# gk969/stm32-speech-recognition

Hardware: AMD Instinct MI355X
Metric: utterances/sec (256-frame, 100 templates) (higher is better)
Workload: dtype int32

## Files before the change

### stm32_speech_recognition_amd/csrc/k_mfcc.hip

```cpp
#include "sr_fft_dev.h"

#include <type_traits>

#ifndef SR_MEL_CHUNKED
#define SR_MEL_CHUNKED 1
#endif

namespace sr {

constexpr int kMfccWaves = 4;
constexpr int kFramesPerWave = 16, kFramesPerWaveMid = 4, kFramesPerWaveSmall = 1;
#ifndef SR_MAG_TAB_BINS
#define SR_MAG_TAB_BINS 8
#endif
constexpr int mfcc_tab_bins(int fpw) { return fpw == kFramesPerWave ? SR_MAG_TAB_BINS : 0; }
static_assert(SR_MAG_TAB_BINS == 0 || SR_MAG_TAB_BINS == 4 || SR_MAG_TAB_BINS == 8, "table bins per lane");
#ifndef SR_MFCC_PIPE
#define SR_MFCC_PIPE 1
#endif
#ifndef SR_MFCC_PIPE_PEEL
#define SR_MFCC_PIPE_PEEL 1
#endif
#ifndef SR_MFCC_PIPE_VMCNT
#define SR_MFCC_PIPE_VMCNT (SR_MFCC_PIPE_PEEL ? 3 : 0)
#endif
static_assert(SR_MFCC_PIPE_VMCNT == 0 || (SR_MFCC_PIPE_VMCNT == 3 && SR_MFCC_PIPE_PEEL), "younger loads counted by the wait");
constexpr bool mfcc_pipelined(int fpw) { return SR_MFCC_PIPE && mfcc_tab_bins(fpw) == 8; }
#ifndef SR_MFCC_TM_REGS
#define SR_MFCC_TM_REGS 1
#endif
#ifdef SR_INJECT_LDS_RACE
#undef SR_MFCC_TM_REGS
#define SR_MFCC_TM_REGS 0
#endif
constexpr bool mfcc_tm_regs(int fpw) { return SR_MFCC_TM_REGS && mfcc_pipelined(fpw); }
constexpr int kMelPad = kMel + 1;
__device__ __forceinline__ constexpr int mel_chunk_word(int j) { return 256 * ((j >> 2) & 1) + 4 * ((j >> 3) ^ (4 * ((j >> 2) & 1))) + (j & 3); }
#ifndef SR_MFCC_PREFIX_TID
#define SR_MFCC_PREFIX_TID 1
#endif
__device__ __forceinline__ constexpr int mel_prefix_word(int j)
{
#if SR_MFCC_PREFIX_TID
    return 64 * (j & 7) + (j >> 3);
#elif SR_MEL_CHUNKED
    return mel_chunk_word(j);
#else
    return j;
#endif
}
#pragma clang diagnostic push
#pragma clang diagnostic ignored "-Winline-asm"
__device__ __forceinline__ void mel_prefix_store(uint32_t base, const uint32_t (&pe)[8], const uint32_t (&po)[8])
{
    static_assert(kBins == 512, "the offsets below are written out for two halves of 512 words");
    asm volatile("s_mov_b32 m0, %16\n\ts_nop 0\n\t"
                 "ds_write_addtid_b32 %0\n\tds_write_addtid_b32 %1 offset:256\n\tds_write_addtid_b32 %2 offset:512\n\t"
                 "ds_write_addtid_b32 %3 offset:768\n\tds_write_addtid_b32 %4 offset:1024\n\tds_write_addtid_b32 %5 offset:1280\n\t"
                 "ds_write_addtid_b32 %6 offset:1536\n\tds_write_addtid_b32 %7 offset:1792\n\t"
                 "ds_write_addtid_b32 %8 offset:2048\n\tds_write_addtid_b32 %9 offset:2304\n\tds_write_addtid_b32 %10 offset:2560\n\t"
                 "ds_write_addtid_b32 %11 offset:2816\n\tds_write_addtid_b32 %12 offset:3072\n\tds_write_addtid_b32 %13 offset:3328\n\t"
                 "ds_write_addtid_b32 %14 offset:3584\n\tds_write_addtid_b32 %15 offset:3840"
                 :
                 : "v"(pe[0]), "v"(pe[1]), "v"(pe[2]), "v"(pe[3]), "v"(pe[4]), "v"(pe[5]), "v"(pe[6]), "v"(pe[7]), "v"(po[0]),
                   "v"(po[1]), "v"(po[2]), "v"(po[3]), "v"(po[4]), "v"(po[5]), "v"(po[6]), "v"(po[7]), "s"(base)
                 : "m0", "memory");
}
#pragma clang diagnostic pop
constexpr int mfcc_wave_lds_words(int fpw) { return kXchgWords + fpw * kMelPad + 64; }

template <typename Base>
struct MfccTabArgs : Base {
    const uint16_t *mag_q;
    uint32_t mag_table_off;
};
template <typename Base>
constexpr int mfcc_feat_kind<MfccTabArgs<Base>> = mfcc_feat_kind<Base>;
template <typename Base>
static MfccTabArgs<Base> mfcc_tab_args(const Base &b, const MfccMagTab &tab)
{
    MfccTabArgs<Base> r;
    static_cast<Base &>(r) = b;
    r.mag_q = tab.mag_q;
    r.mag_table_off = tab.mag_table_off;
    return r;
}

template <int kFPW, typename Args = MfccTabArgs<MfccArgs>>
__global__ void __launch_bounds__(64 * kMfccWaves, 4) k_mfcc(const Args a)
{
    constexpr int kFeat = mfcc_feat_kind<Args>;
    constexpr uint32_t kFeatW = (kFeat == SR_FEAT_FFT || kFeat == SR_FEAT_MAG) ? kBins : kMel;
    constexpr int kWaveLdsWords = mfcc_wave_lds_words(kFPW);
    constexpr int kTabBins = mfcc_tab_bins(kFPW);
    constexpr bool kPipe = mfcc_pipelined(kFPW);
    constexpr bool kTmRegs = mfcc_tm_regs(kFPW);
    extern __shared__ __attribute__((aligned(16))) uint32_t smem[];
    __shared__ uint32_t s_dctM[kCoef * kMelPad];
    __shared__ int s_dctS[kCoef * kMelPad];
    __shared__ u32x4 s_tw3[kTw3Row * 4], s_tw5[8 * 64];
    __shared__ u32x4 s_tm[4 * 64];
    const int lane = threadIdx.x & 63, w = __builtin_amdgcn_readfirstlane(threadIdx.x >> 6);
    uint32_t *buf = smem + w * kWaveLdsWords;
    uint32_t *xw = buf;
    uint32_t *powb = buf + kXchgWords, *moff = powb + kFPW * kMelPad;
    const uint32_t buf_lds = (uint32_t)(uintptr_t)(const __attribute__((address_space(3))) uint32_t *)buf;
    (void)buf_lds;

    for (int i = threadIdx.x; i < kCoef * kMel; i += blockDim.x) {
        const int c = a.t.dct[i], o = (i / kMel) * kMelPad + i % kMel;
        s_dctM[o] = (uint32_t)(((c < 0 ? -c : c) * 262144 + 99) / 100);
        s_dctS[o] = (c > 0) - (c < 0);
    }
    __syncthreads();

    LaneTw tw;
    load_lane_tw(a.t, lane, tw);
    real_leg_tw(tw);
    if (w == 0 && lane < 4) {
        const uint32_t *f = &tw.s3[0][0][0];
#pragma unroll
        for (int c = 0; c < 8; c++) s_tw3[lane * kTw3Row + c] = u32x4{f[4 * c], f[4 * c + 1], f[4 * c + 2], f[4 * c + 3]};
    }
    if (w == 1 % kMfccWaves) store_tw32(s_tw5, lane, tw.s5);
    u32x4 tm_r[4];
    if constexpr (kTmRegs) {
#pragma unroll
        for (int c = 0; c < 2; c++) {
            tm_r[c] = *(const u32x4 *)(a.t.tri_even_m + 8 * lane + 4 * c);
            tm_r[c + 2] = *(const u32x4 *)(a.t.tri_odd_m + 8 * lane + 4 * c);
        }
    }
#ifndef SR_INJECT_LDS_RACE
    if (!kTmRegs && w == 2 % kMfccWaves) {
#pragma unroll
        for (int c = 0; c < 2; c++) {
            s_tm[64 * c + lane] = *(const u32x4 *)(a.t.tri_even_m + 8 * lane + 4 * c);
            s_tm[64 * (c + 2) + lane] = *(const u32x4 *)(a.t.tri_odd_m + 8 * lane + 4 * c);
        }
    }
#endif
    __syncthreads();
#ifdef SR_INJECT_LDS_RACE
    if (w == 2 % kMfccWaves) {
#if SR_INJECT_LDS_RACE >= 2
        __builtin_amdgcn_s_sleep(127);
#endif
#pragma unroll
        for (int c = 0; c < 2; c++) {
            s_tm[64 * c + lane] = *(const u32x4 *)(a.t.tri_even_m + 8 * lane + 4 * c);
            s_tm[64 * (c + 2) + lane] = *(const u32x4 *)(a.t.tri_odd_m + 8 * lane + 4 * c);
        }
    }
#endif
    int hamm_m[3];
#pragma unroll
    for (int k = 0; k < 3; k++) hamm_m[k] = (lane + 64 * k < kFrameLen) ? hamm_fused_multiplier(a.t.hamm[lane + 64 * k]) : 0;
    int f_lo = 0, p_hi = 0, p_lo = 0, x_hi = 0, x_lo = 0;
    if (lane < kMel) {
        const int h = lane;
        f_lo = (h == 0) ? 0 : (int)a.t.tri_cen[h - 1];
        const int f_hi = (h == kMel - 1) ? kBins : (int)a.t.tri_cen[h + 1];
        const int ih = f_hi - 1, il = f_lo ? f_lo - 1 : 0, half = (h & 1) ? kBins : 0;
        p_hi = half + mel_prefix_word(ih), x_hi = (ih >> 3) > 0 ? (ih >> 3) - 1 : 0;
        p_lo = half + mel_prefix_word(il), x_lo = (il >> 3) > 0 ? (il >> 3) - 1 : 0;
    }
    const uint64_t mag_p = (uint64_t)a.mag_q;
    const u32x4 mag_rs = {(uint32_t)mag_p, (uint32_t)(mag_p >> 32) | (2u << 16), kMagTabEntries, 0x00027000u};
    const uint32_t tw_off = 32u * (uint32_t)lane;
#if SR_MEL_CHUNKED
    const int e_base = mel_chunk_word(lane);
    constexpr int kEs = 32, kEh = 128;
    const int c0 = mel_chunk_word(8 * lane), c1 = mel_chunk_word(8 * lane + 4);
#else
    const int e_base = lane;
    constexpr int kEs = 64, kEh = 256;
    const int c0 = 8 * lane, c1 = 8 * lane + 4;
#endif

    uint32_t item = blockIdx.x;
    uint32_t nx_nfrm = 0;
    int nx_mid = 0, nx_seg0 = 0;
    if (item < a.n_items) {
        const sr_vad_rec *rec = a.vad + item / a.tiles;
        nx_nfrm = rec->frm_num;
        nx_mid = (int)rec->atap.mid_val;
        nx_seg0 = rec->seg[0];
    }
    for (; item < a.n_items; item += gridDim.x) {
        const uint32_t b = item / a.tiles, tile = item - b * a.tiles;
        const uint32_t nfrm = nx_nfrm;
        const int mid = nx_mid, seg0 = nx_seg0;
        if (item + gridDim.x < a.n_items) {
            const sr_vad_rec *rec = a.vad + (item + gridDim.x) / a.tiles;
            nx_nfrm = rec->frm_num;
            nx_mid = (int)rec->atap.mid_val;
            nx_seg0 = rec->seg[0];
        }
        const uint16_t *row = a.pcm + (uint64_t)b * a.pcm_stride;
        int16_t *out = a.mfcc + (uint64_t)b * a.max_frames * kCoef;
        const uint32_t f0 = tile * (kMfccWaves * kFPW) + w * kFPW;
        uint32_t *frow = nullptr;
        if constexpr (kFeat != 0) frow = a.feat + (uint64_t)b * a.max_frames * kFeatW;
        uint32_t nf = 0;
        if (f0 < nfrm) nf = (nfrm - f0 < (uint32_t)kFPW) ? nfrm - f0 : (uint32_t)kFPW;

        uint32_t s_pp[3] = {0, 0, 0};
        if (nf) {
            const uint16_t *x = row + seg0 + (int)kHop * (int)f0;
#pragma unroll
            for (int k = 0; k < 3; k++) {
                const int i = lane + 64 * k;
                if (i < kFrameLen) s_pp[k] = *(const u32_align2 *)(x + i - 1);
            }
        }
        auto store_prefixes = [&](const uint32_t (&pe)[8], const uint32_t (&po)[8]) {
#if SR_MFCC_PREFIX_TID
            mel_prefix_store(buf_lds, pe, po);
#else
            *(uint4 *)(buf + c0) = make_uint4(pe[0], pe[1], pe[2], pe[3]);
            *(uint4 *)(buf + c1) = make_uint4(pe[4], pe[5], pe[6], pe[7]);
            *(uint4 *)(buf + kBins + c0) = make_uint4(po[0], po[1], po[2], po[3]);
            *(uint4 *)(buf + kBins + c1) = make_uint4(po[4], po[5], po[6], po[7]);
#endif
        };
        if constexpr (!kPipe)
        for (uint32_t fi = 0; fi < nf; fi++) {
#pragma unroll
            for (int k = 0; k < 3; k++) {
                const int i = lane + 64 * k;
                if (i < kFrameLen) k == 0 ? window_store<0>(xw, i, s_pp[k], mid, hamm_m[k]) : window_store<1>(xw, i, s_pp[k], mid, hamm_m[k]);
            }
            if (fi + 1 < nf) {
                const uint16_t *x = row + seg0 + (int)kHop * (int)(f0 + fi + 1);
#pragma unroll
                for (int k = 0; k < 3; k++) {
                    const int i = lane + 64 * k;
                    if (i < kFrameLen) s_pp[k] = *(const u32_align2 *)(x + i - 1);
                }
            }
            wave_sync();
            uint32_t v[4][4], u[4][4];
            fft_front_real160(xw, lane, tw, s_tw3, v);
            fft_exchange(buf, lane, v, u);
#pragma unroll
            for (int e4 = 0; e4 < 4; e4++) fft_pass4_dbl(u, e4, tw);
            wave_sync();
            uint32_t k5[4][4][2];
            load_tw32(s_tw5, lane, k5);
            uint32_t nn[8];
#pragma unroll
            for (int e3 = 0; e3 < 4; e3++) {
                bfly_pk_dbl<true, false, 0>(u[e3][0], u[e3][1], u[e3][2], u[e3][3], k5[e3][0][0], k5[e3][0][1], k5[e3][1][0],
                                            k5[e3][1][1], k5[e3][2][0], k5[e3][2][1], k5[e3][3][0], k5[e3][3][1]);
                if constexpr (kFeat == SR_FEAT_FFT) {
                    uint32_t *fr = frow + (f0 + fi) * kFeatW + lane + 64 * e3;
                    fr[0] = u[e3][0];
                    fr[256] = u[e3][1];
                }
                nn[2 * e3] = (uint32_t)sdot2z(u[e3][0], u[e3][0]);
                nn[2 * e3 + 1] = (uint32_t)sdot2z(u[e3][1], u[e3][1]);
            }
            const uint32_t nmax = max(max(max(max(nn[0], nn[1]), nn[2]), max(max(nn[3], nn[4]), nn[5])), max(nn[6], nn[7]));
#ifdef SR_TESTING
            const bool quiet = __builtin_expect(__builtin_amdgcn_ballot_w64(nmax > kMagSmallMax) == 0 && !a.mag_table_off, 1);
#else
            const bool quiet = __builtin_expect(__builtin_amdgcn_ballot_w64(nmax > kMagSmallMax) == 0, 1);
#endif
            u32x4 tw_e[2], tw_o[2];
            bool cheap = true;
            if (!quiet) {
#pragma unroll
                for (int c = 0; c < 2; c++) {
                    tw_e[c] = *(const u32x4 *)((const char *)a.t.tri_even32 + tw_off + 16 * c);
                    tw_o[c] = *(const u32x4 *)((const char *)a.t.tri_odd32 + tw_off + 16 * c);
                }
                cheap = __builtin_amdgcn_ballot_w64(nmax > a.mag_cheap_max) == 0;
            } else {
                asm volatile("" : "=v"(tw_e[0]), "=v"(tw_e[1]), "=v"(tw_o[0]), "=v"(tw_o[1]));
            }
            uint32_t *eb = buf + e_base;
            if (kTabBins > 0 && quiet) {
                uint32_t tq[8];
#pragma unroll
                for (int e3 = 0; e3 < 4; e3++) {
                    if constexpr (kTabBins == 8)
                        asm volatile("buffer_load_ushort %0, %1, %2, 0 idxen" : "=v"(tq[2 * e3]) : "v"(nn[2 * e3]), "s"(mag_rs));
                    asm volatile("buffer_load_ushort %0, %1, %2, 0 idxen" : "=v"(tq[2 * e3 + 1]) : "v"(nn[2 * e3 + 1]), "s"(mag_rs));
                }
                uint32_t q0s[4];
                if constexpr (kTabBins == 4) {
#pragma unroll
                    for (int e3 = 0; e3 < 4; e3++) q0s[e3] = cvt_u32(__builtin_amdgcn_sqrtf((float)(int)nn[2 * e3]) * 10.0f) << 2;
                }
                if constexpr (kTabBins == 8)
                    asm volatile("s_waitcnt vmcnt(0)" : "+v"(tq[0]), "+v"(tq[1]), "+v"(tq[2]), "+v"(tq[3]), "+v"(tq[4]), "+v"(tq[5]), "+v"(tq[6]), "+v"(tq[7]));
                else
                    asm volatile("s_waitcnt vmcnt(0)" : "+v"(tq[1]), "+v"(tq[3]), "+v"(tq[5]), "+v"(tq[7]));
#pragma unroll
                for (int e3 = 0; e3 < 4; e3++) {
                    uint32_t q0, q1 = tq[2 * e3 + 1];
                    if constexpr (kTabBins == 8) q0 = tq[2 * e3];
                    else q0 = q0s[e3];
                    if constexpr (kFeat == SR_FEAT_MAG) {
                        uint32_t *fr = frow + (f0 + fi) * kFeatW + lane + 64 * e3;
                        fr[0] = q0 >> 2;
                        fr[256] = q1 >> 2;
                    }
                    eb[kEs * e3] = umul24(q0, q0);
                    eb[kEs * e3 + kEh] = umul24(q1, q1);
                }
            } else if (cheap) {
#pragma unroll
                for (int e3 = 0; e3 < 4; e3++) {
                    const f32x2 m = f32x2{__builtin_amdgcn_sqrtf((float)(int)nn[2 * e3]), __builtin_amdgcn_sqrtf((float)(int)nn[2 * e3 + 1])} *
                                    f32x2{10.0f, 10.0f};
                    const uint32_t m0 = cvt_u32(m.x), m1 = cvt_u32(m.y);
                    if constexpr (kFeat == SR_FEAT_MAG) {
                        uint32_t *fr = frow + (f0 + fi) * kFeatW + lane + 64 * e3;
                        fr[0] = m0;
                        fr[256] = m1;
                    }
                    eb[kEs * e3] = umul24(m0, m0);
                    eb[kEs * e3 + kEh] = umul24(m1, m1);
                }
            } else {
#pragma unroll
                for (int e3 = 0; e3 < 4; e3++) {
                    const f32x2 m = sqrt_rn_int2(f32x2{(float)(int)nn[2 * e3], (float)(int)nn[2 * e3 + 1]}) * f32x2{10.0f, 10.0f};
                    const uint32_t m0 = cvt_u32(m.x), m1 = cvt_u32(m.y);
                    if constexpr (kFeat == SR_FEAT_MAG) {
                        uint32_t *fr = frow + (f0 + fi) * kFeatW + lane + 64 * e3;
                        fr[0] = m0;
                        fr[256] = m1;
                    }
                    eb[kEs * e3] = umul24(m0, m0);
                    eb[kEs * e3 + kEh] = umul24(m1, m1);
                }
            }
            wave_sync();
            uint32_t pe[8], po[8], xe, xo;
            {
                const uint4 q0 = *(const uint4 *)(buf + c0), q1 = *(const uint4 *)(buf + c1);
                const uint32_t e[8] = {q0.x, q0.y, q0.z, q0.w, q1.x, q1.y, q1.z, q1.w};
                uint32_t se = 0, so = 0;
                if (quiet) {
#pragma unroll
                    for (int c = 0; c < 2; c++) {
                        const u32x4 me = s_tm[64 * c + lane], mo = s_tm[64 * (c + 2) + lane];
#pragma unroll
                        for (int k = 0; k < 4; k++) {
                            const uint32_t es = kTabBins > 0 ? e[4 * c + k] : e[4 * c + k] << 4;
                            se += mel_term_fused(es, me[k]);
                            so += mel_term_fused(es, mo[k]);
                            pe[4 * c + k] = se;
                            po[4 * c + k] = so;
                        }
                    }
                } else {
#pragma unroll
                    for (int c = 0; c < 2; c++) {
#pragma unroll
                        for (int k = 0; k < 4; k++) {
                            se += e[4 * c + k] * tw_e[c][k] / 100u;
                            so += e[4 * c + k] * tw_o[c][k] / 100u;
                            pe[4 * c + k] = se;
                            po[4 * c + k] = so;
                        }
                    }
                }
                xe = wave_scan_incl(se);
                xo = wave_scan_incl(so);
            }
            store_prefixes(pe, po);
            buf[2 * kBins + lane] = xe;
            moff[lane] = xo;
            wave_sync();
            if (lane < kMel) {
                const uint32_t *X = (lane & 1) ? moff : buf + 2 * kBins;
                const uint32_t hi = buf[p_hi] + X[x_hi], lo = f_lo ? buf[p_lo] + X[x_lo] : 0u;
                powb[fi * kMelPad + lane] = hi - lo;
                if constexpr (kFeat == SR_FEAT_MEL) frow[(f0 + fi) * kFeatW + lane] = hi - lo;
            }
            wave_sync();
        } else {
            uint32_t mq[8] = {0, 0, 0, 0, 0, 0, 0, 0};
            bool pq = true;
            auto window = [&]() {
#pragma unroll
                for (int k = 0; k < 3; k++) {
                    const int i = lane + 64 * k;
                    if (i < kFrameLen) k == 0 ? window_store<0>(xw, i, s_pp[k], mid, hamm_m[k]) : window_store<1>(xw, i, s_pp[k], mid, hamm_m[k]);
                }
            };
            auto request = [&](uint32_t f) {
                const uint16_t *x = row + seg0 + (int)kHop * (int)(f0 + f);
#pragma unroll
                for (int k = 0; k < 3; k++) {
                    const int i = lane + 64 * k;
                    if (i < kFrameLen) s_pp[k] = *(const u32_align2 *)(x + i - 1);
                }
            };
            auto middle = [&](uint32_t fi, uint32_t (&v)[4][4], bool more) {
                uint32_t u[4][4];
                fft_exchange(buf, lane, v, u);
#pragma unroll
                for (int e4 = 0; e4 < 4; e4++) fft_pass4_dbl(u, e4, tw);
                wave_sync();
                uint32_t k5[4][4][2];
                load_tw32(s_tw5, lane, k5);
                uint32_t nn[8];
#pragma unroll
                for (int e3 = 0; e3 < 4; e3++) {
                    bfly_pk_dbl<true, false, 0>(u[e3][0], u[e3][1], u[e3][2], u[e3][3], k5[e3][0][0], k5[e3][0][1], k5[e3][1][0],
                                                k5[e3][1][1], k5[e3][2][0], k5[e3][2][1], k5[e3][3][0], k5[e3][3][1]);
                    if constexpr (kFeat == SR_FEAT_FFT) {
                        uint32_t *fr = frow + (f0 + fi) * kFeatW + lane + 64 * e3;
                        fr[0] = u[e3][0];
                        fr[256] = u[e3][1];
                    }
                    nn[2 * e3] = (uint32_t)sdot2z(u[e3][0], u[e3][0]);
                    nn[2 * e3 + 1] = (uint32_t)sdot2z(u[e3][1], u[e3][1]);
                }
                const uint32_t nmax = max(max(max(max(nn[0], nn[1]), nn[2]), max(max(nn[3], nn[4]), nn[5])), max(nn[6], nn[7]));
                if (more) {
                    wave_sync();
                    window();
                }
#ifdef SR_TESTING
                const bool quiet = __builtin_expect(__builtin_amdgcn_ballot_w64(nmax > kMagSmallMax) == 0 && !a.mag_table_off, 1);
#else
                const bool quiet = __builtin_expect(__builtin_amdgcn_ballot_w64(nmax > kMagSmallMax) == 0, 1);
#endif
                if (quiet) {
#pragma unroll
                    for (int k = 0; k < 8; k++) asm volatile("buffer_load_ushort %0, %1, %2, 0 idxen" : "=v"(mq[k]) : "v"(nn[k]), "s"(mag_rs));
                } else if (__builtin_amdgcn_ballot_w64(nmax > a.mag_cheap_max) == 0) {
#pragma unroll
                    for (int e3 = 0; e3 < 4; e3++) {
                        const f32x2 m = f32x2{__builtin_amdgcn_sqrtf((float)(int)nn[2 * e3]), __builtin_amdgcn_sqrtf((float)(int)nn[2 * e3 + 1])} *
                                        f32x2{10.0f, 10.0f};
                        mq[2 * e3] = cvt_u32(m.x);
                        mq[2 * e3 + 1] = cvt_u32(m.y);
                    }
                } else {
#pragma unroll
                    for (int e3 = 0; e3 < 4; e3++) {
                        const f32x2 m = sqrt_rn_int2(f32x2{(float)(int)nn[2 * e3], (float)(int)nn[2 * e3 + 1]}) * f32x2{10.0f, 10.0f};
                        mq[2 * e3] = cvt_u32(m.x);
                        mq[2 * e3 + 1] = cvt_u32(m.y);
                    }
                }
                pq = quiet;
                if (fi + 2 < nf) request(fi + 2);
            };
            auto back_end = [&](uint32_t r, auto young) {
                wave_sync();
                auto energies = [&]() {
                    uint32_t *eb = buf + e_base;
#pragma unroll
                    for (int e3 = 0; e3 < 4; e3++) {
                        const uint32_t q0 = mq[2 * e3], q1 = mq[2 * e3 + 1];
                        if constexpr (kFeat == SR_FEAT_MAG) {
                            uint32_t *fr = frow + (f0 + r) * kFeatW + lane + 64 * e3;
                            const uint32_t sh = pq ? 2u : 0u;
                            fr[0] = q0 >> sh;
                            fr[256] = q1 >> sh;
                        }
                        eb[kEs * e3] = umul24(q0, q0);
                        eb[kEs * e3 + kEh] = umul24(q1, q1);
                    }
                    wave_sync();
                };
                uint32_t pe[8], po[8], se = 0, so = 0;
                if (pq) {
                    if constexpr (decltype(young)::value)
                        asm volatile("s_waitcnt vmcnt(3)" : "+v"(mq[0]), "+v"(mq[1]), "+v"(mq[2]), "+v"(mq[3]), "+v"(mq[4]), "+v"(mq[5]), "+v"(mq[6]), "+v"(mq[7]));
                    else
                        asm volatile("s_waitcnt vmcnt(0)" : "+v"(mq[0]), "+v"(mq[1]), "+v"(mq[2]), "+v"(mq[3]), "+v"(mq[4]), "+v"(mq[5]), "+v"(mq[6]), "+v"(mq[7]));
                    energies();
                    const uint4 q0 = *(const uint4 *)(buf + c0), q1 = *(const uint4 *)(buf + c1);
                    const uint32_t e[8] = {q0.x, q0.y, q0.z, q0.w, q1.x, q1.y, q1.z, q1.w};
#pragma unroll
                    for (int c = 0; c < 2; c++) {
                        u32x4 me, mo;
                        if constexpr (kTmRegs) me = tm_r[c], mo = tm_r[c + 2];
                        else me = s_tm[64 * c + lane], mo = s_tm[64 * (c + 2) + lane];
#pragma unroll
                        for (int k = 0; k < 4; k++) {
                            se += mel_term_fused(e[4 * c + k], me[k]);
                            so += mel_term_fused(e[4 * c + k], mo[k]);
                            pe[4 * c + k] = se;
                            po[4 * c + k] = so;
                        }
                    }
                } else {
                    u32x4 tw_e[2], tw_o[2];
                    uint32_t off = tw_off;
                    asm("" : "+v"(off));
#pragma unroll
                    for (int c = 0; c < 2; c++) {
                        tw_e[c] = *(const u32x4 *)((const char *)a.t.tri_even32 + off + 16 * c);
                        tw_o[c] = *(const u32x4 *)((const char *)a.t.tri_odd32 + off + 16 * c);
                    }
                    energies();
                    const uint4 q0 = *(const uint4 *)(buf + c0), q1 = *(const uint4 *)(buf + c1);
                    const uint32_t e[8] = {q0.x, q0.y, q0.z, q0.w, q1.x, q1.y, q1.z, q1.w};
#pragma unroll
                    for (int c = 0; c < 2; c++) {
#pragma unroll
                        for (int k = 0; k < 4; k++) {
                            se += e[4 * c + k] * tw_e[c][k] / 100u;
                            so += e[4 * c + k] * tw_o[c][k] / 100u;
                            pe[4 * c + k] = se;
                            po[4 * c + k] = so;
                        }
                    }
                }
                const uint32_t xe = wave_scan_incl(se), xo = wave_scan_incl(so);
                store_prefixes(pe, po);
                buf[2 * kBins + lane] = xe;
                moff[lane] = xo;
                wave_sync();
                if (lane < kMel) {
                    const uint32_t *X = (lane & 1) ? moff : buf + 2 * kBins;
                    const uint32_t hi = buf[p_hi] + X[x_hi], lo = f_lo ? buf[p_lo] + X[x_lo] : 0u;
                    powb[r * kMelPad + lane] = hi - lo;
                    if constexpr (kFeat == SR_FEAT_MEL) frow[(f0 + r) * kFeatW + lane] = hi - lo;
                }
                wave_sync();
            };
            constexpr std::false_type kDrain{};
            if (nf) {
                window();
                if (nf > 1) request(1);
#if SR_MFCC_PIPE_PEEL
                constexpr std::integral_constant<bool, SR_MFCC_PIPE_VMCNT != 0> kSteady{};
                {
                    wave_sync();
                    uint32_t v[4][4];
                    fft_front_real160(xw, lane, tw, s_tw3, v);
                    middle(0, v, nf > 1);
                }
                for (uint32_t fi = 1; fi + 1 < nf; fi++) {
                    wave_sync();
                    uint32_t v[4][4];
                    fft_front_real160(xw, lane, tw, s_tw3, v);
                    back_end(fi - 1, kSteady);
                    middle(fi, v, true);
                }
                if (nf > 1) {
                    wave_sync();
                    uint32_t v[4][4];
                    fft_front_real160(xw, lane, tw, s_tw3, v);
                    back_end(nf - 2, kDrain);
                    middle(nf - 1, v, false);
                }
#else
                for (uint32_t fi = 0; fi < nf; fi++) {
                    wave_sync();
                    uint32_t v[4][4];
                    fft_front_real160(xw, lane, tw, s_tw3, v);
                    if (fi > 0) back_end(fi - 1, kDrain);
                    middle(fi, v, fi + 1 < nf);
                }
#endif
                back_end(nf - 1, kDrain);
            }
        }

        {
            constexpr int kLogRounds = (kFPW * kMelPad + 63) / 64;
            const uint32_t n_log = nf * kMelPad;
            uint32_t nv[kLogRounds], mv[kLogRounds];
            u32x2 tv[kLogRounds];
#pragma unroll
            for (int r = 0; r < kLogRounds; r++) {
                const uint32_t t = lane + 64u * r;
                nv[r] = powb[t];
                mv[r] = log100_est(nv[r]);
                tv[r] = *(const u32_pair_align4 *)((const char *)a.t.log_thr + 4u * mv[r]);
            }
#pragma unroll
            for (int r = 0; r < kLogRounds; r++) {
                const uint32_t t = lane + 64u * r;
                if (t < n_log) powb[t] = log100_fix(nv[r], mv[r], tv[r].x, tv[r].y) << 14;
            }
        }
        wave_sync();
        if constexpr (kFeat == SR_FEAT_LOGMEL) {
            uint32_t *fw = frow + f0 * kFeatW;
            for (uint32_t t = lane; t < nf * kFeatW; t += 64) {
                const uint32_t fi = t / kFeatW, h = t - fi * kFeatW;
                fw[t] = powb[fi * kMelPad + h] >> 14;
            }
        }
        {
            int16_t *out_w = out + (size_t)f0 * kCoef;
#pragma unroll
            for (uint32_t tl = lane; tl < (uint32_t)(kFPW * kCoef); tl += 64) {
                uint32_t t = tl;
                if constexpr (kPipe) asm volatile("" : "+v"(t));
                if (t < nf * kCoef) {
                    const uint32_t fi = umul24(t, 10923u) >> 17, h = t - umul24(fi, (uint32_t)kCoef);
                    const uint32_t *pw = powb + umul24(fi, (uint32_t)kMelPad), *dm = s_dctM + umul24(h, (uint32_t)kMelPad);
                    const int *ds = s_dctS + umul24(h, (uint32_t)kMelPad);
                    int acc = 0;
#pragma unroll
                    for (int i = 0; i < kMel; i++) acc = mad24((int)__umulhi(pw[i], dm[i]), ds[i], acc);
                    out_w[t] = (int16_t)acc;
                }
            }
        }
        wave_sync();
        {
            const uint32_t r0 = f0 + nf, r1 = (f0 + kFPW < a.max_frames) ? f0 + kFPW : a.max_frames;
            for (uint32_t t = r0 * kCoef + lane; t < r1 * kCoef && r0 < r1; t += 64) out[t] = 0;
        }
        if constexpr (kFeat != 0) {
            const uint32_t r0 = f0 + nf, r1 = (f0 + kFPW < a.max_frames) ? f0 + kFPW : a.max_frames;
            for (uint32_t t = r0 * kFeatW + lane; t < r1 * kFeatW && r0 < r1; t += 64) frow[t] = 0;
        }
    }
}

uint32_t mfcc_ext_frames_per_tile();
int mfcc_ext_occupancy(int *per_cu);
void launch_mfcc_ext(const MfccArgs &a, uint32_t grid, hipStream_t s);
void launch_mfcc_ext_features(const MfccArgs &a, int kind, uint32_t *feat, uint32_t grid, hipStream_t s);

uint32_t mfcc_frames_per_tile(uint32_t frame_len) { return frame_len == 320 ? mfcc_ext_frames_per_tile() : (uint32_t)(kMfccWaves * kFramesPerWave); }
uint32_t mfcc_frames_per_tile_small(uint32_t frame_len, uint32_t which)
{
    return frame_len == 320 ? mfcc_ext_frames_per_tile() : (uint32_t)(kMfccWaves * (which ? kFramesPerWaveSmall : kFramesPerWaveMid));
}

uint32_t mfcc_resident_workgroups(uint32_t frame_len)
{
    int dev = 0, n_cu = 0, per_cu = 0;
    if (hipGetDevice(&dev) != hipSuccess) return 0;
    if (hipDeviceGetAttribute(&n_cu, hipDeviceAttributeMultiprocessorCount, dev) != hipSuccess || n_cu < 1) return 0;
    int e;
    if (frame_len == 320)
        e = mfcc_ext_occupancy(&per_cu);
    else
        e = (int)hipOccupancyMaxActiveBlocksPerMultiprocessor(&per_cu, k_mfcc<kFramesPerWave>, 64 * kMfccWaves,
                                                              (size_t)kMfccWaves * mfcc_wave_lds_words(kFramesPerWave) * sizeof(uint32_t));
    if (e != (int)hipSuccess || per_cu < 1) return 0;
    return (uint32_t)(per_cu * n_cu);
}

void launch_mfcc(const MfccArgs &a, const MfccMagTab &tab, hipStream_t s)
{
    if (a.generic) {
        launch_mfcc_gen(a, s);
        return;
    }
    if (a.n_items == 0) return;
    const uint32_t cap = a.grid_cap ? a.grid_cap : 4096u;
    const uint32_t grid = a.n_items < cap ? a.n_items : cap;
    if (a.frame_len == 320) {
        launch_mfcc_ext(a, grid, s);
        return;
    }
    if (a.small_tiles == 2) {
        const size_t lds = (size_t)kMfccWaves * mfcc_wave_lds_words(kFramesPerWaveSmall) * sizeof(uint32_t);
        SR_LAUNCH_POINT(s, "k_mfcc");
        hipLaunchKernelGGL(k_mfcc<kFramesPerWaveSmall>, dim3(grid), dim3(64 * kMfccWaves), lds, s, mfcc_tab_args(a, tab));
        return;
    }
    if (a.small_tiles == 1) {
        const size_t lds = (size_t)kMfccWaves * mfcc_wave_lds_words(kFramesPerWaveMid) * sizeof(uint32_t);
        SR_LAUNCH_POINT(s, "k_mfcc");
        hipLaunchKernelGGL(k_mfcc<kFramesPerWaveMid>, dim3(grid), dim3(64 * kMfccWaves), lds, s, mfcc_tab_args(a, tab));
        return;
    }
    const size_t lds = (size_t)kMfccWaves * mfcc_wave_lds_words(kFramesPerWave) * sizeof(uint32_t);
    SR_LAUNCH_POINT(s, "k_mfcc");
    hipLaunchKernelGGL(k_mfcc<kFramesPerWave>, dim3(grid), dim3(64 * kMfccWaves), lds, s, mfcc_tab_args(a, tab));
}

template <int kFPW, int kKind>
static void launch_mfcc_feat_kind(const MfccArgs &a, const MfccMagTab &tab, uint32_t *feat, uint32_t grid, hipStream_t s)
{
    const size_t lds = (size_t)kMfccWaves * mfcc_wave_lds_words(kFPW) * sizeof(uint32_t);
    SR_LAUNCH_POINT(s, "k_mfcc");
    hipLaunchKernelGGL((k_mfcc<kFPW, MfccTabArgs<MfccFeatArgs<kKind>>>), dim3(grid), dim3(64 * kMfccWaves), lds, s,
                       mfcc_tab_args(mfcc_feat_args<kKind>(a, feat), tab));
}
template <int kFPW>
static void launch_mfcc_feat_form(const MfccArgs &a, const MfccMagTab &tab, int kind, uint32_t *feat, uint32_t grid, hipStream_t s)
{
    switch (kind) {
    case SR_FEAT_FFT: launch_mfcc_feat_kind<kFPW, SR_FEAT_FFT>(a, tab, feat, grid, s); break;
    case SR_FEAT_MAG: launch_mfcc_feat_kind<kFPW, SR_FEAT_MAG>(a, tab, feat, grid, s); break;
    case SR_FEAT_MEL: launch_mfcc_feat_kind<kFPW, SR_FEAT_MEL>(a, tab, feat, grid, s); break;
    case SR_FEAT_LOGMEL: launch_mfcc_feat_kind<kFPW, SR_FEAT_LOGMEL>(a, tab, feat, grid, s); break;
    default: break;
    }
}

void launch_mfcc_features(const MfccArgs &a, const MfccMagTab &tab, int kind, uint32_t *feat, hipStream_t s)
{
    if (a.generic) {
        launch_mfcc_gen_features(a, kind, feat, s);
        return;
    }
    if (a.n_items == 0) return;
    const uint32_t cap = a.grid_cap ? a.grid_cap : 4096u;
    const uint32_t grid = a.n_items < cap ? a.n_items : cap;
    if (a.frame_len == 320)
        launch_mfcc_ext_features(a, kind, feat, grid, s);
    else if (a.small_tiles == 2)
        launch_mfcc_feat_form<kFramesPerWaveSmall>(a, tab, kind, feat, grid, s);
    else if (a.small_tiles == 1)
        launch_mfcc_feat_form<kFramesPerWaveMid>(a, tab, kind, feat, grid, s);
    else
        launch_mfcc_feat_form<kFramesPerWave>(a, tab, kind, feat, grid, s);
}

}
```

Baseline: 3.467 million.

## Restructure MFCC wave loop with cross-item request, carry and scalar record loads

Factors the log/DCT/zero-fill tail into an epilogue lambda and adds optional modes that prefetch the next work item's first frame and carry the last frame's back end into the next item, overlapping item boundaries. Those cross-item modes are off by default (NEXT_REQ=0, CARRY=0). The default-on change loads the VAD record through the constant address space so it can go through scalar loads. It also rewrites the peeled pipeline's first frame with explicit exchange store/load and unconditional clamped PCM loads. A debug frame-repeat knob is added. The restructuring adds register pressure and control complexity.

```diff
diff --git a/stm32_speech_recognition_amd/csrc/k_mfcc.hip b/stm32_speech_recognition_amd/csrc/k_mfcc.hip
--- a/stm32_speech_recognition_amd/csrc/k_mfcc.hip
+++ b/stm32_speech_recognition_amd/csrc/k_mfcc.hip
@@ -26,6 +26,21 @@
 #endif
 static_assert(SR_MFCC_PIPE_VMCNT == 0 || (SR_MFCC_PIPE_VMCNT == 3 && SR_MFCC_PIPE_PEEL), "younger loads counted by the wait");
 constexpr bool mfcc_pipelined(int fpw) { return SR_MFCC_PIPE && mfcc_tab_bins(fpw) == 8; }
+#ifndef SR_MFCC_NEXT_REQ
+#define SR_MFCC_NEXT_REQ 0
+#endif
+#ifndef SR_MFCC_CARRY
+#define SR_MFCC_CARRY SR_MFCC_NEXT_REQ
+#endif
+#ifndef SR_MFCC_REC_SCALAR
+#define SR_MFCC_REC_SCALAR 1
+#endif
+#ifndef SR_MFCC_FRAME_REPEAT
+#define SR_MFCC_FRAME_REPEAT 1
+#endif
+static_assert(!SR_MFCC_CARRY || (SR_MFCC_NEXT_REQ && SR_MFCC_PIPE_PEEL), "the carried form starts from the early request of the peeled loop");
+static_assert(SR_MFCC_FRAME_REPEAT >= 1 && (SR_MFCC_FRAME_REPEAT == 1 || (SR_MFCC_PIPE_PEEL && !SR_MFCC_NEXT_REQ)),
+              "frame repeats measure the drained form of the peeled loop");
 #ifndef SR_MFCC_TM_REGS
 #define SR_MFCC_TM_REGS 1
 #endif
@@ -181,22 +196,33 @@
     uint32_t item = blockIdx.x;
     uint32_t nx_nfrm = 0;
     int nx_mid = 0, nx_seg0 = 0;
-    if (item < a.n_items) {
-        const sr_vad_rec *rec = a.vad + item / a.tiles;
-        nx_nfrm = rec->frm_num;
-        nx_mid = (int)rec->atap.mid_val;
-        nx_seg0 = rec->seg[0];
-    }
+    auto fetch_rec = [&](uint32_t it) {
+        const sr_vad_rec *rec = a.vad + it / a.tiles;
+        if constexpr (kPipe && SR_MFCC_REC_SCALAR) {
+            const auto *crec = (const __attribute__((address_space(4))) sr_vad_rec *)(uintptr_t)rec;
+            nx_nfrm = crec->frm_num;
+            nx_mid = (int)crec->atap.mid_val;
+            nx_seg0 = crec->seg[0];
+        } else {
+            nx_nfrm = rec->frm_num;
+            nx_mid = (int)rec->atap.mid_val;
+            nx_seg0 = rec->seg[0];
+        }
+    };
+    if (item < a.n_items) fetch_rec(item);
+    [[maybe_unused]] int have0 = 0, carried = 0;
+    [[maybe_unused]] bool pq = true;
+    [[maybe_unused]] uint32_t mq[8];
+    [[maybe_unused]] uint32_t pv_nf = 0, pv_f0 = 0, *pv_frow = nullptr;
+    [[maybe_unused]] int16_t *pv_out = nullptr;
+    if constexpr (kPipe) asm volatile("" : "=v"(mq[0]), "=v"(mq[1]), "=v"(mq[2]), "=v"(mq[3]), "=v"(mq[4]), "=v"(mq[5]), "=v"(mq[6]), "=v"(mq[7]));
+    uint32_t s_pp[3] = {0, 0, 0};
+    if constexpr (kPipe && SR_MFCC_CARRY) __builtin_amdgcn_s_waitcnt(0x0F70);
     for (; item < a.n_items; item += gridDim.x) {
         const uint32_t b = item / a.tiles, tile = item - b * a.tiles;
         const uint32_t nfrm = nx_nfrm;
         const int mid = nx_mid, seg0 = nx_seg0;
-        if (item + gridDim.x < a.n_items) {
-            const sr_vad_rec *rec = a.vad + (item + gridDim.x) / a.tiles;
-            nx_nfrm = rec->frm_num;
-            nx_mid = (int)rec->atap.mid_val;
-            nx_seg0 = rec->seg[0];
-        }
+        if (item + gridDim.x < a.n_items) fetch_rec(item + gridDim.x);
         const uint16_t *row = a.pcm + (uint64_t)b * a.pcm_stride;
         int16_t *out = a.mfcc + (uint64_t)b * a.max_frames * kCoef;
         const uint32_t f0 = tile * (kMfccWaves * kFPW) + w * kFPW;
@@ -205,13 +231,20 @@
         uint32_t nf = 0;
         if (f0 < nfrm) nf = (nfrm - f0 < (uint32_t)kFPW) ? nfrm - f0 : (uint32_t)kFPW;
 
-        uint32_t s_pp[3] = {0, 0, 0};
-        if (nf) {
+        bool got0 = false, cont = false;
+        if constexpr (kPipe) {
+            got0 = __builtin_amdgcn_readfirstlane(have0) != 0;
+            cont = __builtin_amdgcn_readfirstlane(carried) != 0;
+            have0 = 0;
+        }
+        (void)cont;
+        if (nf && !got0) {
             const uint16_t *x = row + seg0 + (int)kHop * (int)f0;
 #pragma unroll
             for (int k = 0; k < 3; k++) {
                 const int i = lane + 64 * k;
-                if (i < kFrameLen) s_pp[k] = *(const u32_align2 *)(x + i - 1);
+                if constexpr (kPipe) s_pp[k] = *(const u32_align2 *)(x + (i < kFrameLen ? i : lane) - 1);
+                else if (i < kFrameLen) s_pp[k] = *(const u32_align2 *)(x + i - 1);
             }
         }
         auto store_prefixes = [&](const uint32_t (&pe)[8], const uint32_t (&po)[8]) {
@@ -224,6 +257,64 @@
             *(uint4 *)(buf + kBins + c1) = make_uint4(po[4], po[5], po[6], po[7]);
 #endif
         };
+        auto epilogue = [&](int16_t *out_e, uint32_t *frow_e, uint32_t f0_e, uint32_t nf_e) {
+            (void)frow_e;
+            int ln = lane;
+            if constexpr (kPipe) asm volatile("" : "+v"(ln));
+            {
+                constexpr int kLogRounds = (kFPW * kMelPad + 63) / 64;
+                const uint32_t n_log = nf_e * kMelPad;
+                uint32_t nv[kLogRounds], mv[kLogRounds];
+                u32x2 tv[kLogRounds];
+#pragma unroll
+                for (int r = 0; r < kLogRounds; r++) {
+                    const uint32_t t = ln + 64u * r;
+                    nv[r] = powb[t];
+                    mv[r] = log100_est(nv[r]);
+                    tv[r] = *(const u32_pair_align4 *)((const char *)a.t.log_thr + 4u * mv[r]);
+                }
+#pragma unroll
+                for (int r = 0; r < kLogRounds; r++) {
+                    const uint32_t t = ln + 64u * r;
+                    if (t < n_log) powb[t] = log100_fix(nv[r], mv[r], tv[r].x, tv[r].y) << 14;
+                }
+                if constexpr (kPipe && SR_MFCC_CARRY) __builtin_amdgcn_s_waitcnt(0x0F70);
+            }
+            wave_sync();
+            if constexpr (kFeat == SR_FEAT_LOGMEL) {
+                uint32_t *fw = frow_e + f0_e * kFeatW;
+                for (uint32_t t = ln; t < nf_e * kFeatW; t += 64) {
+                    const uint32_t fi = t / kFeatW, h = t - fi * kFeatW;
+                    fw[t] = powb[fi * kMelPad + h] >> 14;
+                }
+            }
+            {
+                int16_t *out_w = out_e + (size_t)f0_e * kCoef;
+#pragma unroll
+                for (uint32_t tl = ln; tl < (uint32_t)(kFPW * kCoef); tl += 64) {
+                    uint32_t t = tl;
+                    if constexpr (kPipe) asm volatile("" : "+v"(t));
+                    if (t < nf_e * kCoef) {
+                        const uint32_t fi = umul24(t, 10923u) >> 17, h = t - umul24(fi, (uint32_t)kCoef);
+                        const uint32_t *pw = powb + umul24(fi, (uint32_t)kMelPad), *dm = s_dctM + umul24(h, (uint32_t)kMelPad);
+                        const int *ds = s_dctS + umul24(h, (uint32_t)kMelPad);
+                        int acc = 0;
+#pragma unroll
+                        for (int i = 0; i < kMel; i++) acc = mad24((int)__umulhi(pw[i], dm[i]), ds[i], acc);
+                        out_w[t] = (int16_t)acc;
+                    }
+                }
+            }
+            wave_sync();
+            {
+                const uint32_t r0 = f0_e + nf_e, r1 = (f0_e + kFPW < a.max_frames) ? f0_e + kFPW : a.max_frames;
+                for (uint32_t t = r0 * kCoef + ln; t < r1 * kCoef && r0 < r1; t += 64) out_e[t] = 0;
+            }
+            if constexpr (kFeat != 0) {
+                const uint32_t r0 = f0_e + nf_e, r1 = (f0_e + kFPW < a.max_frames) ? f0_e + kFPW : a.max_frames;
+                for (uint32_t t = r0 * kFeatW + ln; t < r1 * kFeatW && r0 < r1; t += 64) frow_e[t] = 0;
+            }
+        };
         if constexpr (!kPipe)
         for (uint32_t fi = 0; fi < nf; fi++) {
 #pragma unroll
@@ -384,26 +475,35 @@
             }
             wave_sync();
         } else {
-            uint32_t mq[8] = {0, 0, 0, 0, 0, 0, 0, 0};
-            bool pq = true;
-            auto window = [&]() {
+            constexpr uint32_t kRep = SR_MFCC_FRAME_REPEAT;
+            const uint32_t nfl = nf * kRep;
+            auto frame_of = [&](uint32_t f) { return kRep > 1 ? f % nf : f; };
+            const uint16_t *nx_x = nullptr;
+            uint32_t nx_nf = 0;
+            auto next_item = [&]() {
+                const uint32_t it = item + gridDim.x;
+                if (it < a.n_items) {
+                    const uint32_t nb = it / a.tiles, nf0 = (it - nb * a.tiles) * (kMfccWaves * kFPW) + w * kFPW;
+                    if (nf0 < nx_nfrm) nx_nf = (nx_nfrm - nf0 < (uint32_t)kFPW) ? nx_nfrm - nf0 : (uint32_t)kFPW;
+                    nx_x = a.pcm + (uint64_t)nb * a.pcm_stride + nx_seg0 + (int)kHop * (int)nf0;
+                }
+            };
+            auto window = [&](int wmid) {
 #pragma unroll
                 for (int k = 0; k < 3; k++) {
                     const int i = lane + 64 * k;
-                    if (i < kFrameLen) k == 0 ? window_store<0>(xw, i, s_pp[k], mid, hamm_m[k]) : window_store<1>(xw, i, s_pp[k], mid, hamm_m[k]);
+                    if (i < kFrameLen) k == 0 ? window_store<0>(xw, i, s_pp[k], wmid, hamm_m[k]) : window_store<1>(xw, i, s_pp[k], wmid, hamm_m[k]);
                 }
             };
-            auto request = [&](uint32_t f) {
-                const uint16_t *x = row + seg0 + (int)kHop * (int)(f0 + f);
+            auto request_at = [&](const uint16_t *x) {
 #pragma unroll
                 for (int k = 0; k < 3; k++) {
                     const int i = lane + 64 * k;
-                    if (i < kFrameLen) s_pp[k] = *(const u32_align2 *)(x + i - 1);
+                    s_pp[k] = *(const u32_align2 *)(x + (i < kFrameLen ? i : lane) - 1);
                 }
             };
-            auto middle = [&](uint32_t fi, uint32_t (&v)[4][4], bool more) {
-                uint32_t u[4][4];
-                fft_exchange(buf, lane, v, u);
+            auto request = [&](uint32_t f) { request_at(row + seg0 + (int)kHop * (int)(f0 + frame_of(f))); };
+            auto middle_u = [&](uint32_t fi, uint32_t (&u)[4][4], bool more, int wmid) {
 #pragma unroll
                 for (int e4 = 0; e4 < 4; e4++) fft_pass4_dbl(u, e4, tw);
                 wave_sync();
@@ -415,7 +515,7 @@
                     bfly_pk_dbl<true, false, 0>(u[e3][0], u[e3][1], u[e3][2], u[e3][3], k5[e3][0][0], k5[e3][0][1], k5[e3][1][0],
                                                 k5[e3][1][1], k5[e3][2][0], k5[e3][2][1], k5[e3][3][0], k5[e3][3][1]);
                     if constexpr (kFeat == SR_FEAT_FFT) {
-                        uint32_t *fr = frow + (f0 + fi) * kFeatW + lane + 64 * e3;
+                        uint32_t *fr = frow + (f0 + frame_of(fi)) * kFeatW + lane + 64 * e3;
                         fr[0] = u[e3][0];
                         fr[256] = u[e3][1];
                     }
@@ -425,7 +525,7 @@
                 const uint32_t nmax = max(max(max(max(nn[0], nn[1]), nn[2]), max(max(nn[3], nn[4]), nn[5])), max(nn[6], nn[7]));
                 if (more) {
                     wave_sync();
-                    window();
+                    window(wmid);
                 }
 #ifdef SR_TESTING
                 const bool quiet = __builtin_expect(__builtin_amdgcn_ballot_w64(nmax > kMagSmallMax) == 0 && !a.mag_table_off, 1);
@@ -452,9 +552,38 @@
                     }
                 }
                 pq = quiet;
-                if (fi + 2 < nf) request(fi + 2);
+                const uint16_t *rx = nullptr;
+                if (fi + 2 < nfl) {
+                    rx = row + seg0 + (int)kHop * (int)(f0 + frame_of(fi + 2));
+                } else if (SR_MFCC_NEXT_REQ && fi + 2 == nfl) {
+                    next_item();
+                    if (nx_nf) rx = nx_x, have0 = 1;
+                } else if (SR_MFCC_CARRY && more && nx_nf > 1) {
+                    rx = nx_x + kHop;
+                }
+                if (rx) request_at(rx);
             };
-            auto back_end = [&](uint32_t r, auto young) {
+            auto middle = [&](uint32_t fi, uint32_t (&v)[4][4], bool more, int wmid) {
+                uint32_t u[4][4];
+                fft_exchange(buf, lane, v, u);
+                middle_u(fi, u, more, wmid);
+            };
+            auto xchg_store = [&](const uint32_t (&v)[4][4]) {
+                const int jw = (lane & 3) + 64 * ((lane >> 2) & 3) + 256 * (lane >> 4);
+#pragma unroll
+                for (int d1 = 0; d1 < 4; d1++)
+#pragma unroll
+                    for (int d2 = 0; d2 < 4; d2++) buf[xaddr(jw + 4 * d1 + 16 * d2)] = v[d1][d2];
+            };
+            auto xchg_load = [&](uint32_t (&u)[4][4]) {
+                wave_sync();
+#pragma unroll
+                for (int e3 = 0; e3 < 4; e3++)
+#pragma unroll
+                    for (int e4 = 0; e4 < 4; e4++) u[e3][e4] = buf[xaddr(lane + 64 * e3 + 256 * e4)];
+            };
+            auto back_end = [&](uint32_t r, bool young, uint32_t *frow_b, uint32_t f0_b) {
+                (void)frow_b, (void)f0_b;
                 wave_sync();
                 auto energies = [&]() {
                     uint32_t *eb = buf + e_base;
@@ -462,7 +591,7 @@
                     for (int e3 = 0; e3 < 4; e3++) {
                         const uint32_t q0 = mq[2 * e3], q1 = mq[2 * e3 + 1];
                         if constexpr (kFeat == SR_FEAT_MAG) {
-                            uint32_t *fr = frow + (f0 + r) * kFeatW + lane + 64 * e3;
+                            uint32_t *fr = frow_b + (f0_b + r) * kFeatW + lane + 64 * e3;
                             const uint32_t sh = pq ? 2u : 0u;
                             fr[0] = q0 >> sh;
                             fr[256] = q1 >> sh;
@@ -474,10 +603,10 @@
                 };
                 uint32_t pe[8], po[8], se = 0, so = 0;
                 if (pq) {
-                    if constexpr (decltype(young)::value)
-                        asm volatile("s_waitcnt vmcnt(3)" : "+v"(mq[0]), "+v"(mq[1]), "+v"(mq[2]), "+v"(mq[3]), "+v"(mq[4]), "+v"(mq[5]), "+v"(mq[6]), "+v"(mq[7]));
-                    else
-                        asm volatile("s_waitcnt vmcnt(0)" : "+v"(mq[0]), "+v"(mq[1]), "+v"(mq[2]), "+v"(mq[3]), "+v"(mq[4]), "+v"(mq[5]), "+v"(mq[6]), "+v"(mq[7]));
+                    if (SR_MFCC_PIPE_VMCNT != 0 && young) asm volatile("s_waitcnt vmcnt(3)");
+                    else asm volatile("s_waitcnt vmcnt(0)");
+                    __builtin_amdgcn_sched_barrier(0);
+                    asm volatile("" : "+v"(mq[0]), "+v"(mq[1]), "+v"(mq[2]), "+v"(mq[3]), "+v"(mq[4]), "+v"(mq[5]), "+v"(mq[6]), "+v"(mq[7]));
                     energies();
                     const uint4 q0 = *(const uint4 *)(buf + c0), q1 = *(const uint4 *)(buf + c1);
                     const uint32_t e[8] = {q0.x, q0.y, q0.z, q0.w, q1.x, q1.y, q1.z, q1.w};
@@ -526,101 +655,66 @@
                     const uint32_t *X = (lane & 1) ? moff : buf + 2 * kBins;
                     const uint32_t hi = buf[p_hi] + X[x_hi], lo = f_lo ? buf[p_lo] + X[x_lo] : 0u;
                     powb[r * kMelPad + lane] = hi - lo;
-                    if constexpr (kFeat == SR_FEAT_MEL) frow[(f0 + r) * kFeatW + lane] = hi - lo;
+                    if constexpr (kFeat == SR_FEAT_MEL) frow_b[(f0_b + r) * kFeatW + lane] = hi - lo;
                 }
                 wave_sync();
             };
-            constexpr std::false_type kDrain{};
+            constexpr bool kDrain = false, kSteady = true;
+            bool carry = false;
             if (nf) {
-                window();
-                if (nf > 1) request(1);
 #if SR_MFCC_PIPE_PEEL
-                constexpr std::integral_constant<bool, SR_MFCC_PIPE_VMCNT != 0> kSteady{};
                 {
+                    uint32_t v[4][4];
+                    if (cont) {
+                        wave_sync();
+                        fft_front_real160(xw, lane, tw, s_tw3, v);
+                        back_end(pv_nf - 1, nfl > 1, pv_frow, pv_f0);
+                        xchg_store(v);
+                        epilogue(pv_out, pv_frow, pv_f0, pv_nf);
+                    } else {
+                        window(mid);
+                        if (nfl > 1) request(1);
+                        wave_sync();
+                        fft_front_real160(xw, lane, tw, s_tw3, v);
+                        xchg_store(v);
+                    }
+                    uint32_t u[4][4];
+                    xchg_load(u);
+                    middle_u(0, u, nfl > 1, mid);
+                }
+                for (uint32_t fi = 1; fi + 1 < nfl; fi++) {
                     wave_sync();
                     uint32_t v[4][4];
                     fft_front_real160(xw, lane, tw, s_tw3, v);
-                    middle(0, v, nf > 1);
-                }
-                for (uint32_t fi = 1; fi + 1 < nf; fi++) {
+                    back_end(frame_of(fi - 1), kSteady, frow, f0);
+                    middle(fi, v, true, mid);
+                }
+                if (nfl > 1) {
                     wave_sync();
                     uint32_t v[4][4];
                     fft_front_real160(xw, lane, tw, s_tw3, v);
-                    back_end(fi - 1, kSteady);
-                    middle(fi, v, true);
-                }
-                if (nf > 1) {
-                    wave_sync();
-                    uint32_t v[4][4];
-                    fft_front_real160(xw, lane, tw, s_tw3, v);
-                    back_end(nf - 2, kDrain);
-                    middle(nf - 1, v, false);
+                    const bool nreq = __builtin_amdgcn_readfirstlane(have0) != 0;
+                    back_end(frame_of(nfl - 2), nreq, frow, f0);
+                    carry = SR_MFCC_CARRY && nreq;
+                    middle(nfl - 1, v, carry, nx_mid);
                 }
 #else
+                window(mid);
+                if (nf > 1) request(1);
                 for (uint32_t fi = 0; fi < nf; fi++) {
                     wave_sync();
                     uint32_t v[4][4];
                     fft_front_real160(xw, lane, tw, s_tw3, v);
-                    if (fi > 0) back_end(fi - 1, kDrain);
-                    middle(fi, v, fi + 1 < nf);
-                }
-#endif
-                back_end(nf - 1, kDrain);
-            }
+                    if (fi > 0) back_end(fi - 1, kDrain, frow, f0);
+                    middle(fi, v, fi + 1 < nf, mid);
+                }
+#endif
+                if (!carry) back_end(frame_of(nfl - 1), kDrain, frow, f0);
+            }
+            carried = carry;
+            pv_nf = nf, pv_f0 = f0, pv_frow = frow, pv_out = out;
         }
-
-        {
-            constexpr int kLogRounds = (kFPW * kMelPad + 63) / 64;
-            const uint32_t n_log = nf * kMelPad;
-            uint32_t nv[kLogRounds], mv[kLogRounds];
-            u32x2 tv[kLogRounds];
-#pragma unroll
-            for (int r = 0; r < kLogRounds; r++) {
-                const uint32_t t = lane + 64u * r;
-                nv[r] = powb[t];
-                mv[r] = log100_est(nv[r]);
-                tv[r] = *(const u32_pair_align4 *)((const char *)a.t.log_thr + 4u * mv[r]);
-            }
-#pragma unroll
-            for (int r = 0; r < kLogRounds; r++) {
-                const uint32_t t = lane + 64u * r;
-                if (t < n_log) powb[t] = log100_fix(nv[r], mv[r], tv[r].x, tv[r].y) << 14;
-            }
-        }
-        wave_sync();
-        if constexpr (kFeat == SR_FEAT_LOGMEL) {
-            uint32_t *fw = frow + f0 * kFeatW;
-            for (uint32_t t = lane; t < nf * kFeatW; t += 64) {
-                const uint32_t fi = t / kFeatW, h = t - fi * kFeatW;
-                fw[t] = powb[fi * kMelPad + h] >> 14;
-            }
-        }
-        {
-            int16_t *out_w = out + (size_t)f0 * kCoef;
-#pragma unroll
-            for (uint32_t tl = lane; tl < (uint32_t)(kFPW * kCoef); tl += 64) {
-                uint32_t t = tl;
-                if constexpr (kPipe) asm volatile("" : "+v"(t));
-                if (t < nf * kCoef) {
-                    const uint32_t fi = umul24(t, 10923u) >> 17, h = t - umul24(fi, (uint32_t)kCoef);
-                    const uint32_t *pw = powb + umul24(fi, (uint32_t)kMelPad), *dm = s_dctM + umul24(h, (uint32_t)kMelPad);
-                    const int *ds = s_dctS + umul24(h, (uint32_t)kMelPad);
-                    int acc = 0;
-#pragma unroll
-                    for (int i = 0; i < kMel; i++) acc = mad24((int)__umulhi(pw[i], dm[i]), ds[i], acc);
-                    out_w[t] = (int16_t)acc;
-                }
-            }
-        }
-        wave_sync();
-        {
-            const uint32_t r0 = f0 + nf, r1 = (f0 + kFPW < a.max_frames) ? f0 + kFPW : a.max_frames;
-            for (uint32_t t = r0 * kCoef + lane; t < r1 * kCoef && r0 < r1; t += 64) out[t] = 0;
-        }
-        if constexpr (kFeat != 0) {
-            const uint32_t r0 = f0 + nf, r1 = (f0 + kFPW < a.max_frames) ? f0 + kFPW : a.max_frames;
-            for (uint32_t t = r0 * kFeatW + lane; t < r1 * kFeatW && r0 < r1; t += 64) frow[t] = 0;
-        }
+        if (!carried) epilogue(out, frow, f0, nf);
     }
 }
 
```

Result: no change. 3.483 million (median of 6 runs) (+0.5%).
